# lasgroup/safe-adaptation-gym

Measured on AMD Instinct MI355X. Metric: env-steps/sec (batched) Point/GoToGoal, higher is better.
Workload: dtype f32

## Files before the change

### safe_adaptation_gym_amd/csrc/sag_api.hip

```cpp
#include <hip/hip_runtime.h>

#include <cmath>
#include <cstdarg>
#include <cstdio>
#include <cstdlib>
#include <algorithm>
#include <cstring>
#include <string>
#include <vector>

#include "sag_device.hpp"
#include "sag_reset.hpp"
#include "sag_rollout.hpp"
#include "sag_fork.hpp"

#ifndef SAG_SPLIT_MIN_ENVS
#define SAG_EARLY_FORK_MIN_ENVS 2097152
#define SAG_SPLIT_MIN_ENVS 262144
#define SAG_SPLIT_MIN_ENVS_CAR 393216
#endif

using namespace sag;

namespace {
// ... 340 lines not shown

void launch_lidar_cost(sag_ctx* c, int n, int K, const float* d_robot, const float* d_pts, const uint8_t* d_grp, float hazard_size,
                       float* d_lid, int32_t* d_bins, uint8_t* d_cost) {
  static const bool use_reg = [] { const char* e = getenv("SAG_LIDAR_REG"); return !e || atoi(e) != 0; }();
  int team = n <= 16384 ? 16 : (n <= 262144 ? 8 : 4);
  if (const char* e = getenv("SAG_LIDAR_TEAM")) team = atoi(e);
  if (team == 2)
    hipLaunchKernelGGL(k_lidar_cost_team<2>, dim3((n + 31) / 32), dim3(WAVE), 0, c->stream, n, K, d_robot, d_pts, d_grp, hazard_size,
                       d_lid, d_bins, d_cost);
  else if (team == 8)
    hipLaunchKernelGGL(k_lidar_cost_team<8>, dim3((n + 7) / 8), dim3(WAVE), 0, c->stream, n, K, d_robot, d_pts, d_grp, hazard_size,
                       d_lid, d_bins, d_cost);
  else if (team >= 16)
    hipLaunchKernelGGL(k_lidar_cost_team<16>, dim3((n + 3) / 4), dim3(WAVE), 0, c->stream, n, K, d_robot, d_pts, d_grp, hazard_size,
                       d_lid, d_bins, d_cost);
  else if (team >= 4)
    hipLaunchKernelGGL(k_lidar_cost_team<4>, dim3((n + 15) / 16), dim3(WAVE), 0, c->stream, n, K, d_robot, d_pts, d_grp, hazard_size,
                       d_lid, d_bins, d_cost);
  else if (K <= LC_KREG && use_reg)
    hipLaunchKernelGGL(k_lidar_cost_reg, dim3((n + WAVE - 1) / WAVE), dim3(WAVE), 0, c->stream, n, K, d_robot, d_pts, d_grp,
                       hazard_size, d_lid, d_bins, d_cost);
  else
    hipLaunchKernelGGL(k_lidar_cost, dim3((n + WAVE - 1) / WAVE), dim3(WAVE), lidar_cost_lds_bytes(K), c->stream, n, K, d_robot, d_pts,
                       d_grp, hazard_size, d_lid, d_bins, d_cost);
}

}

extern "C" {

int sag_device_count(void) {
  int n = 0;
  if (hipGetDeviceCount(&n) != hipSuccess) return 0;
  return n;
}

int sag_robot_info(int32_t robot, int32_t out[5], double* dt) {
  if (robot < 0 || robot > 2 || !out || !dt) return SAG_ERR_ARG;
  const RobotInfo& r = ROBOTS[robot];
  out[0] = r.nu; out[1] = r.obs_dim; out[2] = r.nstep; out[3] = r.nq; out[4] = r.nv;
  *dt = r.dt;
  return SAG_OK;
}

const char* sag_last_error(const sag_ctx* ctx) { return ctx ? ctx->err.c_str() : g_create_error.c_str(); }

int sag_create(const sag_config* cfg, sag_ctx** out) {
  if (!cfg || !out) return fail(nullptr, SAG_ERR_ARG, "null argument");
  *out = nullptr;
  if (cfg->abi_version != SAG_ABI_VERSION)
    return fail(nullptr, SAG_ERR_ARG, "ABI version %d, library is %d", cfg->abi_version, SAG_ABI_VERSION);
  if (cfg->robot < 0 || cfg->robot > 2) return fail(nullptr, SAG_ERR_ARG, "bad robot %d", cfg->robot);
  if (cfg->n_envs <= 0) return fail(nullptr, SAG_ERR_ARG, "n_envs must be positive");
  if (cfg->max_hazards < 0 || cfg->max_hazards > SAG_MAX_HAZARDS || cfg->max_vases < 0 ||
      cfg->max_vases > SAG_MAX_VASES || cfg->max_pillars < 0 || cfg->max_pillars > SAG_MAX_PILLARS ||
      cfg->max_buttons < 0 || cfg->max_buttons > SAG_MAX_BUTTONS)
    return fail(nullptr, SAG_ERR_ARG, "capacity out of range");
  int ndev = 0;
  if (hipGetDeviceCount(&ndev) != hipSuccess || ndev == 0)
    return fail(nullptr, SAG_ERR_NODEVICE, "no HIP device visible");
  if (cfg->device < 0 || cfg->device >= ndev)
    return fail(nullptr, SAG_ERR_NODEVICE, "device %d out of range (%d visible)", cfg->device, ndev);
  sag_ctx* c = new sag_ctx();
  c->cfg = *cfg; c->rb = ROBOTS[cfg->robot]; c->N = cfg->n_envs;
  c->split = c->N >= (cfg->robot == SAG_ROBOT_CAR ? SAG_SPLIT_MIN_ENVS_CAR : SAG_SPLIT_MIN_ENVS);
  if (const char* e = getenv("SAG_SPLIT")) c->split = atoi(e) != 0;
  const size_t N = (size_t)c->N;
#define CREATE_CHK(call)                                                                         \
  do {                                                                                           \
    hipError_t e_ = (call);                                                                      \
    if (e_ != hipSuccess) {                                                                      \
      int rc_ = fail(nullptr, SAG_ERR_HIP, "%s failed: %s", #call, hipGetErrorString(e_));       \
      sag_destroy(c);                                                                            \
      return rc_;                                                                                \
    }                                                                                            \
  } while (0)
  CREATE_CHK(hipSetDevice(cfg->device));
  CREATE_CHK(hipStreamCreateWithFlags(&c->stream, hipStreamNonBlocking));
  {
    int lo = 0, hi = 0;
    CREATE_CHK(hipDeviceGetStreamPriorityRange(&lo, &hi));
    CREATE_CHK(hipStreamCreateWithPriority(&c->stream2, hipStreamNonBlocking, lo));
  }
  CREATE_CHK(hipEventCreateWithFlags(&c->ev_fork, hipEventDisableTiming));
  CREATE_CHK(hipEventCreateWithFlags(&c->ev_join, hipEventDisableTiming));
  CREATE_CHK(hipEventCreateWithFlags(&c->ev_xsrc, hipEventDisableTiming));
  CREATE_CHK(hipEventCreateWithFlags(&c->ev_xdone, hipEventDisableTiming));
  if (const char* e = getenv("SAG_EARLY_FORK")) c->early_fork = atoi(e);
  if (const char* e = getenv("SAG_BUSY_KINDS")) c->busy_kinds = atoi(e) != 0 ? 1 : 0;
  if (const char* e = getenv("SAG_BUSY_KINDS_MIN")) c->kinds_min = atoi(e);
  {
    hipDeviceProp_t prop;
    if (hipGetDeviceProperties(&prop, cfg->device) == hipSuccess && prop.multiProcessorCount > 0) c->n_cu = prop.multiProcessorCount;
  }
  CREATE_CHK(hipMalloc(&c->S, N * DEV_FLOATS * sizeof(float)));
  CREATE_CHK(hipMalloc(&c->I, icount(N) * sizeof(int32_t)));
  CREATE_CHK(hipMalloc(&c->G, N * 3 * NBODY * sizeof(float)));
  CREATE_CHK(hipMalloc(&c->d_rows, BUSY_CLASSES * N * sizeof(int32_t)));
  CREATE_CHK(hipMalloc(&c->d_kind, N));
  CREATE_CHK(hipMemset(c->d_kind, 0, N));
  CREATE_CHK(hipMalloc(&c->d_count, (2 * BUSY_CLASSES + 1) * sizeof(int32_t)));
  CREATE_CHK(hipMemset(c->d_count, 0, (2 * BUSY_CLASSES + 1) * sizeof(int32_t)));
  CREATE_CHK(hipMalloc(&c->L_f, N * SAG_REC_FLOATS * sizeof(float)));
  CREATE_CHK(hipMalloc(&c->L_i, N * SAG_REC_INTS * sizeof(int32_t)));
  CREATE_CHK(hipMalloc(&c->st_f, N * SAG_REC_FLOATS * sizeof(float)));
  CREATE_CHK(hipMalloc(&c->st_i, N * SAG_REC_INTS * sizeof(int32_t)));
// ... 748 lines not shown
```

### safe_adaptation_gym_amd/csrc/sag_device.hpp

```cpp
#pragma once
#include <hip/hip_runtime.h>
#include <stdint.h>

#include <type_traits>

#include "../../include/sag.h"

namespace sag {

constexpr int WAVE = 64;

enum { DI_META = 0, DI_TSTATE = 1, DI_STEP = 2, DI_ENVID = 3, DI_FLAGS = 4, DI_COUNT = 5 };
constexpr int FLAG_EPISODE_SHIFT = 8;
__host__ __device__ constexpr size_t ipad(size_t N) { return (N + 3) & ~(size_t)3; }
__host__ __device__ constexpr size_t icount(size_t N) { return ipad(N) + 4 * N; }
__host__ __device__ constexpr size_t iaddr(int w, size_t N, size_t i) {
  return w == DI_TSTATE ? i : ipad(N) + i * 4 + (w == DI_META ? 0 : (w == DI_STEP ? 1 : (w == DI_ENVID ? 2 : 3)));
}

constexpr int DEV_FLOATS = 192, DEV_GROUPS = DEV_FLOATS / 4;
constexpr int DV_POS = 40, DV_VEL = 76, DG_HAZ = 5, DG_POS = 10, DG_PILLARS = 4, DG_BUTTONS = 28;
__host__ __device__ constexpr int didx(int k) {
  return k < 6 ? k
       : k < 9 ? 136 + (k - 6)
// ... 454 lines not shown
    const float ha = a.box ? a.b : a.a;
    const float lax = obx + a.ox * rc - a.oy * rs, lay = oby + a.ox * rs + a.oy * rc;
    const float pbx = a.a * ac + ha * as + SAT_EPS, pby = a.a * as + ha * ac + SAT_EPS;
#pragma unroll
    for (int gb = 0; gb < NB; gb++) {
      const Geom b = shape_geom(shB, gb, vsz, rstatic);
      const float hb = b.box ? b.b : b.a;
      const bool hit = !(fabsf(lbx[gb] - a.ox) > a.a + pax[gb]) && !(fabsf(lby[gb] - a.oy) > ha + pay[gb]) &&
                       !(fabsf(lax - b.ox) > b.a + pbx) && !(fabsf(lay - b.oy) > hb + pby);
      mask |= (mask_t)hit << (8 * ga + gb);
    }
  }
  int n = 0;
  while (mask) {
    const int pbit = (NA > 4 ? __ffsll((unsigned long long)mask) : __ffs((unsigned int)mask)) - 1;
    mask &= mask - 1;
    const int ga = NA > 1 ? pbit >> 3 : 0, gb = NB > 1 ? pbit & 7 : 0;
    const Geom a = shape_geom(SHA, ga, vsz, rstatic);
    Geom b = shape_geom(shB, gb, vsz, rstatic);
    const float ax = A.x + ca * a.ox - sa * a.oy, ay = A.y + sa * a.ox + ca * a.oy;
    const float qx = B.x + cb * b.ox - sb * b.oy, qy = B.y + sb * b.ox + cb * b.oy;
    if (!a.box && !b.box) n += cc_contact(A, B, ax, ay, a.a, qx, qy, b.a, sol);
    else if (!a.box) n += cb_contact(A, B, ax, ay, a.a, qx, qy, cb, sb, b.a, b.b, true, sol);
    else if (!b.box) n += cb_contact(B, A, qx, qy, b.a, ax, ay, ca, sa, a.a, a.b, false, sol);
    else n += bb_contact(A, B, ax, ay, ca, sa, a.a, a.b, qx, qy, cb, sb, b.a, b.b, sol);
  }
  return n;
}
template <int SHA, bool MULTI>
__device__ inline int collide_list(BV& A, float ca, float sa, BV& B, int shB, float cb, float sb, float vsz,
                                   float rstatic, const Sol& sol) {
#ifdef SAG_COLLIDE_REF
  return collide_shapes<true>(A, SHA, ca, sa, B, shB, cb, sb, vsz, rstatic, sol);
#endif
  if constexpr (MULTI) {
    if (shape_ngeom(shB) > 1) return collide_list_nb<SHA, 5>(A, ca, sa, B, SH_BOX, cb, sb, vsz, rstatic, sol);
  }
  if constexpr (SHA != SH_CAR) return collide_shapes<true>(A, SHA, ca, sa, B, shB, cb, sb, vsz, rstatic, sol);
  return collide_list_nb<SHA, 1>(A, ca, sa, B, shB, cb, sb, vsz, rstatic, sol);
}

constexpr int NBODY = SAG_MAX_VASES + 1, BOX_ID = SAG_MAX_VASES;
constexpr int DPOOL = 3;
enum { LS_X = 0, LS_Y = NBODY, LS_YAW = 2 * NBODY, LS_POOL = 3 * NBODY };
constexpr int LDS_SLOTS = LS_POOL + 6 * DPOOL;
constexpr int LDS_FLOATS = LDS_SLOTS * WAVE;
constexpr int CAR_PARK_SLOTS = 23;
enum { CP_FL = 0, CP_F0 = 5, CP_PX = 8, CP_EACC = 11, CP_Q = 16, CP_TAIL = 20 };
#define CPK(j) lds[(LDS_SLOTS + (j)) * WAVE + lane]
constexpr int STG_BASE = LS_YAW * WAVE;

enum { CY_LOAD = 0, CY_ROBOT, CY_RS, CY_RV, CY_VS, CY_VV_BROAD, CY_VV_NARROW, CY_INTEG, CY_WRITEBACK,
       CY_REWARD, CY_RESAMPLE, CY_COST, CY_LIDAR, CY_OBS_STORE, CY_TAIL, CY_N };
#ifdef SAG_WAVE_TIMES
constexpr int WT_MAX = 16384;
static __device__ unsigned long long g_wt[WT_MAX][2];
static __device__ int g_wt_env[WT_MAX][64];
static __device__ unsigned char g_wt_work[WT_MAX][64][8];
static __device__ unsigned short g_wt_trips[WT_MAX][8];
#define WTW(k) do { if (wt_work[k] < 255) wt_work[k]++; } while (0)
__device__ inline int wt_wave_max(int v) { for (int off = 32; off; off >>= 1) v = max(v, __shfl_xor(v, off)); return v; }
#define WTT(k, v) do { wt_trips[k] += (unsigned)wt_wave_max((int)(v)); } while (0)
#else
#define WTW(k) do {} while (0)
#define WTT(k, v) do {} while (0)
#endif
#ifdef SAG_CYCLES
static __device__ unsigned long long g_cyc[3][CY_N + 1];
static __device__ unsigned long long g_cyc_worst[3][CY_N + 1];
static __device__ unsigned long long g_cyc_worst_block[3];
static __device__ unsigned long long g_cyc_hist[3][64];
#define CYC_DECL unsigned long long cyc_acc[CY_N] = {}; unsigned long long cyc_t = __builtin_readcyclecounter();
#define CYC(k) do { const unsigned long long t_ = __builtin_readcyclecounter(); cyc_acc[k] += t_ - cyc_t; cyc_t = t_; } while (0)
__device__ inline unsigned long long cyc_wave_red(unsigned long long v, bool take_max) {
  for (int off = 32; off; off >>= 1) {
    const unsigned long long o = ((unsigned long long)(unsigned)__shfl_xor((int)(v >> 32), off) << 32) | (unsigned)__shfl_xor((int)(v & 0xffffffffu), off);
    v = take_max ? (o > v ? o : v) : (o < v ? o : v);
  }
  return v;
}
#define CYC_FLUSH(mode) do { unsigned long long tot_ = 0, red_[CY_N]; \
    for (int k_ = 0; k_ < CY_N; k_++) { red_[k_] = cyc_wave_red(k_ == CY_ROBOT && !live ? ~0ull : cyc_acc[k_], k_ != CY_ROBOT); tot_ += red_[k_]; } \
    if (lane == 0) { for (int k_ = 0; k_ < CY_N; k_++) atomicAdd(&g_cyc[mode][k_], red_[k_]); \
    atomicAdd(&g_cyc[mode][CY_N], 1ull); \
    { const int lg_ = 63 - __clzll((long long)(tot_ | 1ull)); const int q_ = lg_ >= 2 ? (int)(tot_ >> (lg_ - 2) & 3ull) : 0; \
      const int b_ = 4 * lg_ + q_ - 40; atomicAdd(&g_cyc_hist[mode][b_ < 0 ? 0 : (b_ > 63 ? 63 : b_)], 1ull); } \
    if (atomicMax(&g_cyc_worst[mode][CY_N], tot_) < tot_) { for (int k_ = 0; k_ < CY_N; k_++) g_cyc_worst[mode][k_] = red_[k_]; g_cyc_worst_block[mode] = blockIdx.x; } } } while (0)
#else
#define CYC_DECL
#define CYC(k) do {} while (0)
#define CYC_FLUSH(mode) do {} while (0)
#endif
}
#include "sag_doggo.hpp"
namespace sag {
#define SF(k) S[saddr((k), (size_t)N, (size_t)i)]
#define SD(d) S[((size_t)((d) >> 2) * N + i) * 4 + ((d) & 3)]
#define LP(base, k) lds[((base) + (k)) * WAVE + lane]
#define POOL(d, c) lds[(LS_POOL + (d) * 6 + (c)) * WAVE + lane]
#define STG(j) lds[STG_BASE + lane * STG_STRIDE + (j)]
#define TILE(b) lds[STG_BASE + (b) * WAVE + lane]

constexpr uint32_t TS_AWAKE_SHIFT = 17, TS_AWAKE_BITS = (1u << NBODY) - 1;

struct Dyn {
  float* lds; float* S; float* G; int lane, N, i;
  uint32_t dmap;
  uint32_t ovf;
  int nd;
  __device__ int vel_field(int k) const { return DV_VEL + 3 * k; }
  __device__ int slot(int k) const { return (int)(dmap >> (2 * k) & 3u) - 1; }
  __device__ bool has(int k) const { return (dmap >> (2 * k) & 3u) || (ovf >> k & 1u); }
  __device__ void ensure(int k, bool from_state) {
    if (has(k)) return;
    float vx = 0, vy = 0, w = 0;
    if (nd < DPOOL) {
      if (from_state) { const int f = vel_field(k); vx = SD(f); vy = SD(f + 1); w = SD(f + 2); }
      const int d = nd++;
      dmap |= (uint32_t)(d + 1) << (2 * k);
      POOL(d, 0) = vx; POOL(d, 1) = vy; POOL(d, 2) = w; POOL(d, 3) = 0; POOL(d, 4) = 0; POOL(d, 5) = 0;
    } else {
      ovf |= 1u << k;
      if (!from_state) { const int f = vel_field(k); SD(f) = 0; SD(f + 1) = 0; SD(f + 2) = 0; }
      for (int c = 0; c < 3; c++) G[((size_t)c * NBODY + k) * N + i] = 0;
    }
  }
  __device__ void get(int k, float& vx, float& vy, float& w, float& ax, float& ay, float& aw) const {
    const int d = slot(k);
    if (d >= 0) { vx = POOL(d, 0); vy = POOL(d, 1); w = POOL(d, 2); ax = POOL(d, 3); ay = POOL(d, 4); aw = POOL(d, 5); }
    else if (ovf >> k & 1u) {
      const int f = vel_field(k);
      vx = SD(f); vy = SD(f + 1); w = SD(f + 2);
      ax = G[((size_t)0 * NBODY + k) * N + i]; ay = G[((size_t)1 * NBODY + k) * N + i]; aw = G[((size_t)2 * NBODY + k) * N + i];
    } else { vx = vy = w = ax = ay = aw = 0; }
  }
  __device__ void set_acc(int k, float ax, float ay, float aw) {
    const int d = slot(k);
    if (d >= 0) { POOL(d, 3) = ax; POOL(d, 4) = ay; POOL(d, 5) = aw; }
    else { G[((size_t)0 * NBODY + k) * N + i] = ax; G[((size_t)1 * NBODY + k) * N + i] = ay; G[((size_t)2 * NBODY + k) * N + i] = aw; }
  }
  __device__ void set_vel(int k, float vx, float vy, float w) {
    const int d = slot(k);
    if (d >= 0) { POOL(d, 0) = vx; POOL(d, 1) = vy; POOL(d, 2) = w; }
    else { const int f = vel_field(k); SD(f) = vx; SD(f + 1) = vy; SD(f + 2) = w; }
  }
};

struct BodyK { int sh; float m, I, reff; };

struct LidarHit { int bin; float alias, sensor; };

__device__ __attribute__((noinline)) LidarHit lidar_exact(float rxf, float ryf, float yawf, float px, float py) {
// ... 88 lines not shown
  if (!is_task_obj || bk.sh == SH_BOX) {
    const float mm = !is_task_obj ? vk.m : bk.m, II = !is_task_obj ? vk.I : bk.I, rr = !is_task_obj ? vk.reff : bk.reff;
    const float fmax_ = MU * GRAV * mm;
    float fx = -SOL_D0 * mm * (bc * vx_ + ax_), fy = -SOL_D0 * mm * (bc * vy_ + ay_);
    const float f2 = fx * fx + fy * fy;
    if (f2 > fmax_ * fmax_) { const float sc = fmax_ / sqrtf(f2); fx *= sc; fy *= sc; }
    ax_ += fx / mm; ay_ += fy / mm;
    const float t = clampf(-SOL_D0 * II * (bc * w_ + aw_), -fmax_ * rr, fmax_ * rr);
    aw_ += t / II;
  } else {
    float c, s; sincosf(B[2], &s, &c);
    float bvx = c * vx_ + s * vy_, bvy = -s * vx_ + c * vy_, bax = c * ax_ + s * ay_, bay = -s * ax_ + c * ay_;
    const float mg = bk.m * GRAV;
    float tlim;
    if (bk.sh == SH_ROD) {
      const float mx = 1.5f * bk.m, lx = 0.05f * mg / 0.08f, ly = 1.2f * mg;
      const float fx = clampf(-SOL_D0 * mx * (bc * bvx + bax), -lx, lx);
      const float fy = clampf(-SOL_D0 * bk.m * (bc * bvy + bay), -ly, ly);
      bax += fx / mx; bay += fy / bk.m;
      tlim = 1.2f * mg * 0.15f;
    } else {
      const float me = 1.4f * bk.m, lim = 0.05f * mg / 0.14f;
      float fx = -SOL_D0 * me * (bc * bvx + bax), fy = -SOL_D0 * me * (bc * bvy + bay);
      const float f2 = fx * fx + fy * fy;
      if (f2 > lim * lim) { const float sc = lim / sqrtf(f2); fx *= sc; fy *= sc; }
      bax += fx / me; bay += fy / me;
      tlim = 0.003f * mg;
    }
    ax_ = c * bax - s * bay; ay_ = s * bax + c * bay;
    aw_ += clampf(-SOL_D0 * bk.I * (bc * w_ + aw_), -tlim, tlim) / bk.I;
  }
  vx_ += h * ax_; vy_ += h * ay_; w_ += h * aw_;
  if (fabsf(vx_) < REST_V && fabsf(vy_) < REST_V && fabsf(w_) < REST_W && fabsf(h * ax_) < REST_V &&
      fabsf(h * ay_) < REST_V && fabsf(h * aw_) < REST_W) { vx_ = 0; vy_ = 0; w_ = 0; }
  B[3] = vx_; B[4] = vy_; B[5] = w_;
  B[0] += h * vx_; B[1] += h * vy_; B[2] += h * w_;
}


enum { MODE_ALL = 0, MODE_QUIET = 1, MODE_BUSY = 2, MODE_POST = 3 };

constexpr int obs_dim(int robot) { return robot == SAG_ROBOT_DOGGO ? 104 : (robot == SAG_ROBOT_CAR ? 72 : 60); }
constexpr int quiet_lds_rows_chunked(int robot) { return LS_YAW + (robot == SAG_ROBOT_CAR ? 25 : 17); }
constexpr int quiet_lds_total(int robot) {
  const int own = quiet_lds_rows_chunked(robot) * WAVE * (int)sizeof(float), busy = (LDS_FLOATS + WAVE) * (int)sizeof(float);
  return busy > own ? own + (busy - own + 511) / 512 * 512 : own;
}
constexpr bool obs_whole_rows(int robot, bool has_btn, bool has_tbox, int mode) {
  const int cols = obs_dim(robot) - 16;
  return robot != SAG_ROBOT_DOGGO && mode != MODE_POST && !has_btn && !has_tbox && cols - 16 >= 2 * NBODY &&
         cols <= LDS_SLOTS &&
         cols * WAVE * (int)sizeof(float) <= quiet_lds_total(robot);
}
constexpr int quiet_lds_rows(int robot, bool has_btn, bool has_tbox) {
  const int chunked = quiet_lds_rows_chunked(robot), whole = obs_dim(robot) - 16;
  return obs_whole_rows(robot, has_btn, has_tbox, MODE_QUIET) && whole > chunked ? whole : chunked;
}
constexpr uint32_t TS_BUSY_BIT = 1u << 28;
constexpr int BUSY_CLASSES = 8;
__host__ __device__ constexpr int busy_class_order(int k) {
  constexpr int order[BUSY_CLASSES] = {7, 5, 3, 1, 6, 4, 2, 0};
  return order[k];
}

inline CarFricK car_fric_constants(float h) {
  CarFricK k;
  constexpr float CM = CAR_M, CIO = CAR_IO, COY = CAR_OY, CRW = 0.05f, AB = -CM * COY;
  constexpr float IDC = 1.0f / (CM * (CM * CIO - AB * AB));
  constexpr float M0 = (CM * CIO) * IDC, M2 = (-AB * CM) * IDC, M3 = (CM * CIO - AB * AB) * IDC, M5 = (CM * CM) * IDC;
  k.iIw = 1.0f / (CAR_IW + h * 0.001f); k.iIb = 1.0f / (CAR_IB + h * 0.001f);
  const float spw = CRW * CRW * k.iIw, spb = CRW * CRW * k.iIb;
  const float A_L = M3 + M5 * 0.13f * 0.13f + spw, A_T = M0 - 2 * M2 * 0.1f + M5 * 0.1f * 0.1f;
  const float A_X = M0 + 2 * M2 * 0.1f + M5 * 0.1f * 0.1f + spb, A_Y = M3 + spb;
  constexpr float RF = (1.0f - SOL_D0) / SOL_D0;
  k.R_L = A_L * RF; k.R_T = 0.5f * A_T * RF; k.R_X = A_X * RF; k.R_Y = A_Y * RF;
  k.iA_L = 1.0f / (A_L + k.R_L); k.iA_T = 1.0f / (A_T + k.R_T); k.iA_X = 1.0f / (A_X + k.R_X); k.iA_Y = 1.0f / (A_Y + k.R_Y);
  k.w_L = 1.0f / (spw + k.R_L); k.w_T = 1.0f / k.R_T; k.w_X = 1.0f / (spb + k.R_X); k.w_Y = 1.0f / (spb + k.R_Y);
  k.K00 = CM + k.w_T + k.w_X; k.K02 = AB - 0.1f * k.w_T + 0.1f * k.w_X;
  k.K22 = CIO + 0.13f * 0.13f * (k.w_L + k.w_L) + 0.1f * 0.1f * k.w_T + 0.1f * 0.1f * k.w_X;
  k.idk = 1.0f / (k.K00 * k.K22 - k.K02 * k.K02);
  k.iK11 = 1.0f / (CM + k.w_L + k.w_L + k.w_Y);
  return k;
}

template <int ROBOT, bool HAS_BTN, bool HAS_TBOX, int MODE>
__device__ __forceinline__ void step_body(const StepArgs& p, float* lds, const int lane, const int i,
                                          const bool live, const int base_env, const int nvalid,
                                          const uint64_t skip_mask, const int* rows) {
  constexpr int NSTAT = SAG_MAX_PILLARS + (HAS_BTN ? SAG_MAX_BUTTONS : 0);
  constexpr bool CAR = ROBOT == SAG_ROBOT_CAR, DOGGO = ROBOT == SAG_ROBOT_DOGGO;
  static_assert(!DOGGO || MODE == MODE_ALL || MODE == MODE_POST, "Doggo runs the single-launch form");
  static_assert(DOGGO || MODE != MODE_POST, "MODE_POST is the Doggo post kernel");
  constexpr bool QUIET = MODE == MODE_QUIET;
  constexpr bool PARK = CAR && !QUIET;
  constexpr int SH_ME = CAR ? SH_CAR : SH_ROBOT;
  constexpr int OBS_DIM = DOGGO ? 104 : (CAR ? 72 : 60);
  constexpr int NSENS = DOGGO ? 28 : OBS_DIM - 48, NCHUNK = DOGGO ? 5 : 4;
  constexpr int STG_STRIDE = DOGGO ? 29 : (CAR ? 25 : 17);
  static_assert(STG_BASE + WAVE * STG_STRIDE <= LDS_FLOATS, "staging tile must fit");
  CYC_DECL
  const float my_bound = shape_bound(SH_ME, 0.f, 0.f);
  const int N = p.N;
  float* __restrict__ S = p.S;
  int32_t* __restrict__ I = p.I;
  const int capV = p.max_vases, capH = p.max_hazards, capP = p.max_pillars, capB = HAS_BTN ? p.max_buttons : 0;

  const float4* __restrict__ S4 = reinterpret_cast<const float4*>(S);
  auto G4 = [&](int g) { return S4[(size_t)g * N + i]; };
  const bool use_hot = MODE == MODE_BUSY && p.hot != nullptr;
  const float4* __restrict__ H4 = use_hot ? reinterpret_cast<const float4*>(p.hot) + (size_t)i * HOT_GROUPS : nullptr;
  auto GH = [&](int g, int hslot) { return use_hot ? H4[hslot] : G4(g); };
  int4 iw;
  uint32_t tstate;
  if (use_hot) {
    const float4 hi = H4[14], ht = H4[15];
    iw = make_int4(__float_as_int(hi.x), __float_as_int(hi.y), __float_as_int(hi.z), __float_as_int(hi.w));
    tstate = (uint32_t)__float_as_int(ht.x);
  } else {
    iw = reinterpret_cast<const int4*>(I + ipad((size_t)N))[i];
    tstate = (uint32_t)I[iaddr(DI_TSTATE, (size_t)N, (size_t)i)];
  }
  const uint32_t meta = (uint32_t)iw.x;
  int step = iw.y;
  const uint32_t env_id = (uint32_t)iw.z;
  const float4 gA = GH(0, 0), gB = GH(1, 1), gC = GH(2, 2), gD = GH(3, 3);
  BV R;
  R.x = gA.x; R.y = gA.y;
  float yaw = gA.z;
  R.vx = gA.w; R.vy = gB.x; R.w = gB.y;
  R.ax = R.ay = R.aw = 0; R.dyn = 1;
  const float gear = gC.y, damp = gC.z;
  const float vsz = gD.z, psz = gD.w;
  float ext[9] = {0, 0, 0, 0, 0, 1, 0, 0, 0}, eacc[5] = {0, 0, 0, 0, 0};
  constexpr int DG_EXT = (152 >> 2);
  static_assert(didx(SAG_F_ROBOT_EXT) == 152 && didx(SAG_F_ROBOT_EXT + 8) == 160, "car extension = device groups 38..40");
  float4 ext_tail = make_float4(0.f, 0.f, 0.f, 0.f);
  if constexpr (CAR) {
    const float4 e0 = G4(DG_EXT), e1 = G4(DG_EXT + 1);
    ext_tail = G4(DG_EXT + 2);
    ext[0] = e0.x; ext[1] = e0.y; ext[2] = e0.z; ext[3] = e0.w; ext[4] = e1.x; ext[5] = e1.y; ext[6] = e1.z; ext[7] = e1.w;
    ext[8] = ext_tail.x;
    if constexpr (PARK) {
      CPK(CP_Q) = ext[5]; CPK(CP_Q + 1) = ext[6]; CPK(CP_Q + 2) = ext[7]; CPK(CP_Q + 3) = ext[8];
      CPK(CP_TAIL) = ext_tail.y; CPK(CP_TAIL + 1) = ext_tail.z; CPK(CP_TAIL + 2) = ext_tail.w;
    }
  }
  float goalx = gB.z, goaly = gB.w;
  float last0 = gC.x;
  float a0 = 0, a1 = 0, n0 = 0, n1 = 0;
  if (!p.observe_only) {
    if constexpr (!DOGGO) {
      const float2 a = reinterpret_cast<const float2*>(p.actions)[i];
      a0 = a.x; a1 = a.y;
      if (p.noise) { const float2 z = reinterpret_cast<const float2*>(p.noise)[i]; n0 = z.x; n1 = z.y; }
    }
  }
  {
    float vpos[36];
    const int need = HAS_TBOX && p.has_box ? 9 : (3 * capV + 3) / 4;
#pragma unroll
    for (int g = 0; g < 9; g++) {
      float4 v = make_float4(0.f, 0.f, 0.f, 0.f);
      if (g < need) v = GH(DG_POS + g, 5 + g);
      vpos[4 * g] = v.x; vpos[4 * g + 1] = v.y; vpos[4 * g + 2] = v.z; vpos[4 * g + 3] = v.w;
    }
#pragma unroll
    for (int k = 0; k < SAG_MAX_VASES; k++)
      if (k >= capV) { vpos[3 * k] = vpos[3 * k + 1] = vpos[3 * k + 2] = 0; }
    if (!(HAS_TBOX && p.has_box)) { vpos[3 * BOX_ID] = vpos[3 * BOX_ID + 1] = vpos[3 * BOX_ID + 2] = 0; }
#pragma unroll
    for (int k = 0; k < NBODY; k++) { LP(LS_X, k) = vpos[3 * k]; LP(LS_Y, k) = vpos[3 * k + 1]; LP(LS_YAW, k) = vpos[3 * k + 2]; }
  }
  float stx[NSTAT], sty[NSTAT];
  {
    float4 v = make_float4(0.f, 0.f, 0.f, 0.f);
    if (capP > 0) v = GH(DG_PILLARS, 4);
    stx[0] = v.x; sty[0] = v.y; stx[1] = capP > 1 ? v.z : 0.f; sty[1] = capP > 1 ? v.w : 0.f;
    static_assert(SAG_MAX_PILLARS == 2, "pillars fill one group");
  }
  if constexpr (HAS_BTN) {
    float bt[12];
#pragma unroll
    for (int g = 0; g < 3; g++) {
      float4 v = make_float4(0.f, 0.f, 0.f, 0.f);
      if (2 * g < capB) v = G4(DG_BUTTONS + g);
      bt[4 * g] = v.x; bt[4 * g + 1] = v.y; bt[4 * g + 2] = v.z; bt[4 * g + 3] = v.w;
    }
    static_assert(SAG_MAX_BUTTONS == 6, "buttons fill three groups");
#pragma unroll
    for (int k = 0; k < SAG_MAX_BUTTONS; k++) {
      stx[SAG_MAX_PILLARS + k] = k < capB ? bt[2 * k] : 0.f;
      sty[SAG_MAX_PILLARS + k] = k < capB ? bt[2 * k + 1] : 0.f;
    }
  }
  const int task = meta & 15, nH = meta >> 4 & 15, nV = meta >> 8 & 15, nP = meta >> 12 & 3,
            nB = HAS_BTN ? (meta >> 14 & 7) : 0, box_kind = HAS_TBOX ? (meta >> 17 & 3) : 0;
  const bool has_box = HAS_TBOX && box_kind != SAG_BOX_NONE;
  auto is_box = [](int k) { return HAS_TBOX && k == BOX_ID; };
  int flags = 0;

  Rng rng;
  rng.tape = p.tape ? p.tape + (size_t)i * p.tape_len : nullptr;
  rng.len = p.tape_len; rng.pos = 0; rng.exhausted = 0;
  rng.k0 = p.key0; rng.k1 = p.key1; rng.env = env_id; rng.step = (uint32_t)step;
  rng.ep4 = ((uint32_t)iw.w >> FLAG_EPISODE_SHIFT) << 2;

  float ctrl0 = 0, ctrl1 = 0;
  float ctrl12[DOGGO ? 12 : 1] = {};
  if constexpr (DOGGO) {
    if (!p.observe_only) {
      const float an = SF(SAG_F_ACTION_NOISE);
#pragma unroll 1
      for (int j = 0; j < 12; j += 2) {
        float z0, z1;
        if (p.noise) { z0 = p.noise[(size_t)i * 12 + j]; z1 = p.noise[(size_t)i * 12 + j + 1]; }
        else {
          uint32_t c[4] = {rng.env, rng.step, (uint32_t)(j >> 1), rng.ep4 | 1u};
          philox4x32_10(c, p.key0, p.key1);
          box_muller(c[0], c[1], z0, z1);
        }
        const float l0 = SF(SAG_F_CTRL_SCALE + j), l1 = SF(SAG_F_CTRL_SCALE + j + 1);
        ctrl12[j] = clampf(p.actions[(size_t)i * 12 + j] + an * z0, -l0, l0);
        ctrl12[j + 1] = clampf(p.actions[(size_t)i * 12 + j + 1] + an * z1, -l1, l1);
      }
    }
  }
  if (!p.observe_only) {
    if (!p.noise && !DOGGO) {
      uint32_t c[4] = {rng.env, rng.step, 0u, rng.ep4 | 1u};
      philox4x32_10(c, p.key0, p.key1);
      box_muller(c[0], c[1], n0, n1);
    }
    const float an = gC.w;
    const float cs0 = gD.x, cs1 = gD.y;
    ctrl0 = clampf(a0 + an * n0, -cs0, cs0);
    ctrl1 = clampf(a1 + an * n1, -cs1, cs1);
    if (task == SAG_TASK_CATCH_GOAL) {
      int t = tstate >> 7 & 15;
      t = t - 1 > 0 ? t - 1 : 0;
      float cur = SF(SAG_F_CATCH + 2), nxt = SF(SAG_F_CATCH + 3);
      if (t == 0) {
        cur = nxt;
        nxt = (float)rng.uniform(0.2, 1.0);
        if (rng.exhausted) flags |= 2;
        if (live) { SF(SAG_F_CATCH + 2) = cur; SF(SAG_F_CATCH + 3) = nxt; }
// ... 519 lines not shown
    const float dth = (fmaxf(fabsf(R.w), 3.0f) + 1.0f) * T;
    const float fa = 0.1f + reach, fb = 0.0707107f + reach + 0.1f * dth;
    const float Bx = R.x + 0.1f * cy, By = R.y + 0.1f * sy;
#pragma unroll 1
    for (int k = 0; k < nV; k++) {
      const float vx_ = LP(LS_X, k), vy_ = LP(LS_Y, k);
      const float dx = vx_ - R.x, dyy = vy_ - R.y, rs = rr + vase_r;
      if (dx * dx + dyy * dyy <= rs * rs) {
        if constexpr (FINE) {
          float sv, cv; sincosf(LP(LS_YAW, k), &sv, &cv);
          auto box_d2 = [&](float px, float py) {
            const float wx = px - vx_, wy = py - vy_;
            const float ex = fmaxf(fabsf(cv * wx + sv * wy) - vsz, 0.f), ey = fmaxf(fabsf(cv * wy - sv * wx) - vsz, 0.f);
            return ex * ex + ey * ey;
          };
          busy |= box_d2(R.x, R.y) <= fa * fa || box_d2(Bx, By) <= fb * fb;
        } else busy = true;
      }
    }
    if (has_box) {
      const float dx = LP(LS_X, BOX_ID) - R.x, dyy = LP(LS_Y, BOX_ID) - R.y, rs = rr + box_r;
      near_obj = dx * dx + dyy * dyy <= rs * rs;
    }
#pragma unroll 1
    for (int k = 0; k < n_static; k++) {
      if (k == capP) k = SAG_MAX_PILLARS;
      const bool is_p = k < SAG_MAX_PILLARS;
      const bool on = is_p ? (k < nP) : (k - SAG_MAX_PILLARS < nB);
      const float sr = is_p ? psz : BUTTON_R;
      const float skx = pick(stx, k), sky = pick(sty, k);
      const float dx = skx - R.x, dyy = sky - R.y, rs = rr + sr;
      if constexpr (FINE) {
        const float ex = skx - Bx, ey = sky - By;
        near_static |= on && (dx * dx + dyy * dyy <= (fa + sr) * (fa + sr) || ex * ex + ey * ey <= (fb + sr) * (fb + sr));
      } else near_static |= on && dx * dx + dyy * dyy <= rs * rs;
    }
    const bool near_vase = busy && !moving;
    busy |= near_obj || near_static;
    const uint32_t kind = p.busy_kinds ? (uint32_t)near_obj | (uint32_t)near_static << 1 | (uint32_t)(near_vase || moving) << 2 : 0u;
    const uint32_t nbit = TS_BUSY_BIT << (p.phase ^ 1);
    tstate = busy ? (tstate | nbit) : (tstate & ~nbit);
    if (busy && live && p.kind) p.kind[i] = (uint8_t)kind;
    busy_next = busy;
  }

  CYC(CY_WRITEBACK);
  float hzx[SAG_MAX_HAZARDS], hzy[SAG_MAX_HAZARDS];
  float hsz;
  {
    float hz[20];
#pragma unroll
    for (int g = 0; g < 5; g++) {
      float4 v = make_float4(0.f, 0.f, 0.f, 0.f);
      if (g == 4 || 2 * g < capH) v = use_hot ? reinterpret_cast<const float4*>(p.hot_haz)[(size_t)i * 5 + g] : G4(DG_HAZ + g);
      hz[4 * g] = v.x; hz[4 * g + 1] = v.y; hz[4 * g + 2] = v.z; hz[4 * g + 3] = v.w;
    }
    static_assert(SAG_MAX_HAZARDS == 9, "hazards + size fill five groups");
#pragma unroll
    for (int k = 0; k < SAG_MAX_HAZARDS; k++) { hzx[k] = k < capH ? hz[2 * k] : 0.f; hzy[k] = k < capH ? hz[2 * k + 1] : 0.f; }
    hsz = hz[18];
  }

  bool bad = false;
  {
    float v[6] = {R.x, R.y, yaw, R.vx, R.vy, R.w};
#pragma unroll
    for (int k = 0; k < 6; k++) bad |= !(fabsf(v[k]) <= 1e10f);
    if constexpr (DOGGO) {
      bad |= !(fabs(dgs.pos[2]) <= 1e10) || !(fabs(dgs.vlin[2]) <= 1e10);
      for (int k = 0; k < 4; k++) bad |= !(fabs(dgs.quat[k]) <= 1e10);
      for (int k = 0; k < 3; k++) bad |= !(fabs(dgs.wloc[k]) <= 1e10);
      for (int k = 0; k < DG_NJ; k++) bad |= !(fabs(dgs.q[k]) <= 1e10) || !(fabs(dgs.qd[k]) <= 1e10);
    }
  }

  double rew0 = 0, rew1 = 0;
  int met = 0;
  const double rx = R.x, ry = R.y;
  bool need_goal = false;
  float box_last1 = 0, box_last2 = 0;
  if (!p.observe_only && !bad) {
    if (task == SAG_TASK_PRESS_BUTTONS || task == SAG_TASK_PRESS_BUTTONS_SCARCE) {
      int gb = tstate & 7, bstate = tstate >> 3 & 1, timer = tstate >> 4 & 7;
      double gd = dist2d(rx, ry, SD(112 + 2 * gb), SD(113 + 2 * gb));
      double r = task == SAG_TASK_PRESS_BUTTONS ? (double)last0 - gd : 0.0;
      float last = (float)gd;
      if (btn_mask >> gb & 1) {
        r += 1.0; met = 1;
        gb = (int)(rng.word() & 3u);
        if (rng.exhausted) flags |= 2;
        timer = 5;
        last = (float)dist2d(rx, ry, SD(112 + 2 * gb), SD(113 + 2 * gb));
        bstate = 0;
      }
      if (bstate == 0) {
        if (timer != 0) timer -= 1;
        else { bstate = 1; timer = 5; }
      }
      last0 = last;
      tstate = (tstate & ~127u) | (uint32_t)gb | (uint32_t)bstate << 3 | (uint32_t)timer << 4;
      rew0 = r;
    } else if (task == SAG_TASK_COLLECT) {
      uint32_t act = tstate >> 11 & 63;
      if (act == 0) act = (1u << nB) - 1;
      uint32_t hit = act & btn_mask;
      if (hit) {
        rew0 = 1.0; met = 1;
        act &= ~(hit & (0u - hit));
      }
      tstate = (tstate & ~(63u << 11)) | act << 11;
    } else if (!has_box) {
      double gx = goalx, gy = goaly;
      double dx = rx - gx, dyy = ry - gy, dz = (DOGGO ? (double)(float)dgs.pos[2] : (double)PT_Z) - GOAL_Z;
      double dist = sqrt(dx * dx + dyy * dyy + dz * dz);
// ... 380 lines not shown
  if (live) {
    if (p.reward) {
      float2 r;
      r.x = bad ? -10.0f : (float)rew0; r.y = bad ? 0.0f : (float)rew1;
      reinterpret_cast<float2*>(p.reward)[i] = r;
    }
    if (p.cost) p.cost[i] = (uint8_t)cost;
    if (p.done) p.done[i] = bad ? 1 : 0;
    if (p.goal_met) p.goal_met[i] = (uint8_t)met;
    if (p.tape_used) p.tape_used[i] = rng.pos;
  }
  CYC(CY_TAIL);
  CYC_FLUSH(MODE);
#ifdef SAG_WAVE_TIMES
  if (MODE == MODE_BUSY && blockIdx.x < WT_MAX) {
    g_wt_env[blockIdx.x][lane] = live ? i : -1;
    for (int k = 0; k < 8; k++) g_wt_work[blockIdx.x][lane][k] = (unsigned char)wt_work[k];
    if (lane == 0) for (int k = 0; k < 8; k++) g_wt_trips[blockIdx.x][k] = (unsigned short)wt_trips[k];
  }
#endif
}

template <int ROBOT, bool HAS_BTN, bool HAS_TBOX>
__global__ __launch_bounds__(WAVE, SAG_STEP_MIN_WAVES) void k_step(StepArgs p) {
  __shared__ float lds[LDS_FLOATS + (ROBOT == SAG_ROBOT_CAR ? CAR_PARK_SLOTS * WAVE : 0)];
  static_assert(ROBOT != SAG_ROBOT_DOGGO, "Doggo: k_doggo_physics + k_step_doggo_post");
  const int epw = p.envs_per_wave;
  const int lane = threadIdx.x, base = blockIdx.x * epw, gi = base + lane;
  const bool live = gi < p.N && lane < epw;
  step_body<ROBOT, HAS_BTN, HAS_TBOX, MODE_ALL>(p, lds, lane, live ? gi : p.N - 1, live, base,
                                                 min(epw, p.N - base), 0ull, nullptr);
}

template <bool HAS_BTN, bool HAS_TBOX>
__global__ __launch_bounds__(WAVE, 1) void k_step_doggo_post(StepArgs p) {
  __shared__ float lds[LDS_FLOATS];
  const int lane = threadIdx.x, base = blockIdx.x * WAVE, gi = base + lane;
  const bool live = gi < p.N;
  step_body<SAG_ROBOT_DOGGO, HAS_BTN, HAS_TBOX, MODE_POST>(p, lds, lane, live ? gi : p.N - 1, live, base, min(WAVE, p.N - base),
                                                            0ull, nullptr);
}

#ifndef SAG_QUIET_MIN_WAVES
#define SAG_QUIET_MIN_WAVES 4
#endif
#ifndef SAG_CAR_QUIET_MIN_WAVES
#define SAG_CAR_QUIET_MIN_WAVES 3
#endif
template <int ROBOT, bool HAS_BTN, bool HAS_TBOX>
__global__ __launch_bounds__(WAVE, ROBOT == SAG_ROBOT_CAR ? SAG_CAR_QUIET_MIN_WAVES : SAG_QUIET_MIN_WAVES) void k_step_quiet(StepArgs p) {
  constexpr int QSLOTS = quiet_lds_rows(ROBOT, HAS_BTN, HAS_TBOX);
  static_assert(QSLOTS >= LS_YAW + NBODY, "the yaw rows written at load time must stay in bounds");
  static_assert(QSLOTS * WAVE * (int)sizeof(float) <= quiet_lds_total(ROBOT), "the quiet array stays inside the footprint of its launch");
  __shared__ float lds[QSLOTS * WAVE];
  const int lane = threadIdx.x, base = blockIdx.x * WAVE, gi = base + lane;
  const bool in = gi < p.N;
  const bool busy = in && ((uint32_t)p.I[iaddr(DI_TSTATE, (size_t)p.N, (size_t)gi)] & (TS_BUSY_BIT << p.phase));
  const uint64_t skip = __ballot(busy || !in);
  if (skip == ~0ull) return;
  const bool live = in && !busy;
  step_body<ROBOT, HAS_BTN, HAS_TBOX, MODE_QUIET>(p, lds, lane, in ? gi : p.N - 1, live, base,
                                                   min(WAVE, p.N - base), skip, nullptr);
}

constexpr int COMPACT_PER_LANE = 16, COMPACT_ENVS = 256 * COMPACT_PER_LANE;
template <bool KINDS>
__global__ __launch_bounds__(256) void k_compact(const int32_t* I, const uint8_t* kind, int N, int phase, int32_t* rows, int32_t* count,
                                                  int32_t* zero_for_next, const int32_t* prev_total, int kinds_min) {
  constexpr int NC = KINDS ? BUSY_CLASSES : 1;
  const bool use_kinds = KINDS && *prev_total > kinds_min;
  if (blockIdx.x == 0 && threadIdx.x < BUSY_CLASSES) zero_for_next[threadIdx.x] = 0;
  __shared__ int wave_tot[4][BUSY_CLASSES];
  __shared__ int wave_base[4][BUSY_CLASSES];
  const int lane = threadIdx.x & 63, wv = threadIdx.x >> 6;
  const int e0 = blockIdx.x * COMPACT_ENVS + wv * (WAVE * COMPACT_PER_LANE);
  uint32_t bmask = 0;
  uint64_t kinds = 0;
  int pre[COMPACT_PER_LANE];
  int run[BUSY_CLASSES] = {};
  uint32_t tw[COMPACT_PER_LANE];
  uint8_t kb[COMPACT_PER_LANE];
#pragma unroll
  for (int j = 0; j < COMPACT_PER_LANE; j++) {
    const int e = e0 + j * WAVE + lane;
    tw[j] = e < N ? (uint32_t)I[iaddr(DI_TSTATE, (size_t)N, (size_t)e)] : 0u;
    kb[j] = KINDS && e < N && use_kinds ? kind[e] : (uint8_t)0;
  }
#pragma unroll
  for (int j = 0; j < COMPACT_PER_LANE; j++) {
    const bool b = (tw[j] & (TS_BUSY_BIT << phase)) != 0;
    const int k = b ? (int)kb[j] & (BUSY_CLASSES - 1) : 0;
    bmask |= (uint32_t)b << j;
    kinds |= (uint64_t)k << (4 * j);
    pre[j] = 0;
#pragma unroll
    for (int c = 0; c < NC; c++) {
      const uint64_t m = __ballot(b && k == c);
      if (b && k == c) pre[j] = run[c] + __popcll(m & ((1ull << lane) - 1));
      run[c] += __popcll(m);
    }
  }
  if (lane == 0)
#pragma unroll
    for (int c = 0; c < NC; c++) wave_tot[wv][c] = run[c];
  __syncthreads();
  if (threadIdx.x < NC) {
    const int c = threadIdx.x;
    const int total = wave_tot[0][c] + wave_tot[1][c] + wave_tot[2][c] + wave_tot[3][c];
    int base = total ? atomicAdd(count + c, total) : 0;
// ... 490 lines not shown
```

Measured before the change: 4.834 billion.

## Issue quiet Point kernel loads before busy check and park hazards in LDS

```diff
diff --git a/safe_adaptation_gym_amd/csrc/sag_api.hip b/safe_adaptation_gym_amd/csrc/sag_api.hip
--- a/safe_adaptation_gym_amd/csrc/sag_api.hip
+++ b/safe_adaptation_gym_amd/csrc/sag_api.hip
@@ -416,6 +416,7 @@
     return fail(nullptr, SAG_ERR_ARG, "ABI version %d, library is %d", cfg->abi_version, SAG_ABI_VERSION);
   if (cfg->robot < 0 || cfg->robot > 2) return fail(nullptr, SAG_ERR_ARG, "bad robot %d", cfg->robot);
   if (cfg->n_envs <= 0) return fail(nullptr, SAG_ERR_ARG, "n_envs must be positive");
+  if (cfg->n_envs > (1 << 28)) return fail(nullptr, SAG_ERR_ARG, "n_envs above 2^28 is not supported");
   if (cfg->max_hazards < 0 || cfg->max_hazards > SAG_MAX_HAZARDS || cfg->max_vases < 0 ||
       cfg->max_vases > SAG_MAX_VASES || cfg->max_pillars < 0 || cfg->max_pillars > SAG_MAX_PILLARS ||
       cfg->max_buttons < 0 || cfg->max_buttons > SAG_MAX_BUTTONS)
diff --git a/safe_adaptation_gym_amd/csrc/sag_device.hpp b/safe_adaptation_gym_amd/csrc/sag_device.hpp
--- a/safe_adaptation_gym_amd/csrc/sag_device.hpp
+++ b/safe_adaptation_gym_amd/csrc/sag_device.hpp
@@ -530,6 +530,7 @@
 
 enum { CY_LOAD = 0, CY_ROBOT, CY_RS, CY_RV, CY_VS, CY_VV_BROAD, CY_VV_NARROW, CY_INTEG, CY_WRITEBACK,
        CY_REWARD, CY_RESAMPLE, CY_COST, CY_LIDAR, CY_OBS_STORE, CY_TAIL, CY_N };
+enum { CY_Q_HEAD = CY_RS, CY_Q_HAZ = CY_RV };
 #ifdef SAG_WAVE_TIMES
 constexpr int WT_MAX = 16384;
 static __device__ unsigned long long g_wt[WT_MAX][2];
@@ -550,6 +551,7 @@
 static __device__ unsigned long long g_cyc_hist[3][64];
 #define CYC_DECL unsigned long long cyc_acc[CY_N] = {}; unsigned long long cyc_t = __builtin_readcyclecounter();
 #define CYC(k) do { const unsigned long long t_ = __builtin_readcyclecounter(); cyc_acc[k] += t_ - cyc_t; cyc_t = t_; } while (0)
+#define CYC_ARRIVED(v) asm volatile("" :: "v"(v))
 __device__ inline unsigned long long cyc_wave_red(unsigned long long v, bool take_max) {
   for (int off = 32; off; off >>= 1) {
     const unsigned long long o = ((unsigned long long)(unsigned)__shfl_xor((int)(v >> 32), off) << 32) | (unsigned)__shfl_xor((int)(v & 0xffffffffu), off);
@@ -567,6 +569,7 @@
 #else
 #define CYC_DECL
 #define CYC(k) do {} while (0)
+#define CYC_ARRIVED(v) do {} while (0)
 #define CYC_FLUSH(mode) do {} while (0)
 #endif
 }
@@ -576,6 +579,7 @@
 #define SD(d) S[((size_t)((d) >> 2) * N + i) * 4 + ((d) & 3)]
 #define LP(base, k) lds[((base) + (k)) * WAVE + lane]
 #define POOL(d, c) lds[(LS_POOL + (d) * 6 + (c)) * WAVE + lane]
+#define HZP(j) (*((j) < HAZ_PARK_STATIC ? &lds[(LS_POOL + (j)) * WAVE + lane] : &hz_dyn[((j) - HAZ_PARK_STATIC) * WAVE + lane]))
 #define STG(j) lds[STG_BASE + lane * STG_STRIDE + (j)]
 #define TILE(b) lds[STG_BASE + (b) * WAVE + lane]
 
@@ -770,6 +774,12 @@
          cols <= LDS_SLOTS &&
          cols * WAVE * (int)sizeof(float) <= quiet_lds_total(robot);
 }
+constexpr int HAZ_PARK_ROWS = 2 * SAG_MAX_HAZARDS + 1;
+constexpr int HAZ_PARK_STATIC = obs_dim(SAG_ROBOT_POINT) - 16 - LS_POOL;
+constexpr bool quiet_one_phase(int robot, bool has_btn, bool has_tbox) {
+  return robot == SAG_ROBOT_POINT && obs_whole_rows(robot, has_btn, has_tbox, MODE_QUIET) && HAZ_PARK_STATIC > 0 &&
+         (obs_dim(robot) - 16 + HAZ_PARK_ROWS - HAZ_PARK_STATIC) * WAVE * (int)sizeof(float) <= quiet_lds_total(robot);
+}
 constexpr int quiet_lds_rows(int robot, bool has_btn, bool has_tbox) {
   const int chunked = quiet_lds_rows_chunked(robot), whole = obs_dim(robot) - 16;
   return obs_whole_rows(robot, has_btn, has_tbox, MODE_QUIET) && whole > chunked ? whole : chunked;
@@ -803,13 +813,14 @@
 
 template <int ROBOT, bool HAS_BTN, bool HAS_TBOX, int MODE>
 __device__ __forceinline__ void step_body(const StepArgs& p, float* lds, const int lane, const int i,
-                                          const bool live, const int base_env, const int nvalid,
-                                          const uint64_t skip_mask, const int* rows) {
+                                          const bool live_arg, const int base_env, const int nvalid,
+                                          const uint64_t skip_arg, const int* rows) {
   constexpr int NSTAT = SAG_MAX_PILLARS + (HAS_BTN ? SAG_MAX_BUTTONS : 0);
   constexpr bool CAR = ROBOT == SAG_ROBOT_CAR, DOGGO = ROBOT == SAG_ROBOT_DOGGO;
   static_assert(!DOGGO || MODE == MODE_ALL || MODE == MODE_POST, "Doggo runs the single-launch form");
   static_assert(DOGGO || MODE != MODE_POST, "MODE_POST is the Doggo post kernel");
   constexpr bool QUIET = MODE == MODE_QUIET;
+  constexpr bool ONE_PHASE = QUIET && quiet_one_phase(ROBOT, HAS_BTN, HAS_TBOX);
   constexpr bool PARK = CAR && !QUIET;
   constexpr int SH_ME = CAR ? SH_CAR : SH_ROBOT;
   constexpr int OBS_DIM = DOGGO ? 104 : (CAR ? 72 : 60);
@@ -824,7 +835,15 @@
   const int capV = p.max_vases, capH = p.max_hazards, capP = p.max_pillars, capB = HAS_BTN ? p.max_buttons : 0;
 
   const float4* __restrict__ S4 = reinterpret_cast<const float4*>(S);
-  auto G4 = [&](int g) { return S4[(size_t)g * N + i]; };
+  const uint32_t voff = (uint32_t)i << 4;
+  auto G4 = [&](int g) {
+    if constexpr (ONE_PHASE) return *reinterpret_cast<const float4*>(reinterpret_cast<const char*>(S4 + (size_t)g * N) + voff);
+    else return S4[(size_t)g * N + i];
+  };
+  auto G4sel = [&](bool on, int g) {
+    const float4 v = G4(on ? g : 0);
+    return on ? v : make_float4(0.f, 0.f, 0.f, 0.f);
+  };
   const bool use_hot = MODE == MODE_BUSY && p.hot != nullptr;
   const float4* __restrict__ H4 = use_hot ? reinterpret_cast<const float4*>(p.hot) + (size_t)i * HOT_GROUPS : nullptr;
   auto GH = [&](int g, int hslot) { return use_hot ? H4[hslot] : G4(g); };
@@ -834,6 +853,10 @@
     const float4 hi = H4[14], ht = H4[15];
     iw = make_int4(__float_as_int(hi.x), __float_as_int(hi.y), __float_as_int(hi.z), __float_as_int(hi.w));
     tstate = (uint32_t)__float_as_int(ht.x);
+  } else if constexpr (ONE_PHASE) {
+    tstate = *reinterpret_cast<const uint32_t*>(reinterpret_cast<const char*>(I) + (voff >> 2));
+    iw = *reinterpret_cast<const int4*>(reinterpret_cast<const char*>(I + ipad((size_t)N)) + voff);
+    static_assert(iaddr(DI_TSTATE, 8, 5) == 5, "TSTATE is the plain [N] column in front");
   } else {
     iw = reinterpret_cast<const int4*>(I + ipad((size_t)N))[i];
     tstate = (uint32_t)I[iaddr(DI_TSTATE, (size_t)N, (size_t)i)];
@@ -868,31 +891,38 @@
   float a0 = 0, a1 = 0, n0 = 0, n1 = 0;
   if (!p.observe_only) {
     if constexpr (!DOGGO) {
-      const float2 a = reinterpret_cast<const float2*>(p.actions)[i];
+      float2 a;
+      if constexpr (ONE_PHASE) a = *reinterpret_cast<const float2*>(reinterpret_cast<const char*>(p.actions) + (voff >> 1));
+      else a = reinterpret_cast<const float2*>(p.actions)[i];
       a0 = a.x; a1 = a.y;
       if (p.noise) { const float2 z = reinterpret_cast<const float2*>(p.noise)[i]; n0 = z.x; n1 = z.y; }
     }
   }
+  float vpos[36];
   {
-    float vpos[36];
     const int need = HAS_TBOX && p.has_box ? 9 : (3 * capV + 3) / 4;
 #pragma unroll
     for (int g = 0; g < 9; g++) {
       float4 v = make_float4(0.f, 0.f, 0.f, 0.f);
-      if (g < need) v = GH(DG_POS + g, 5 + g);
+      if constexpr (ONE_PHASE) v = G4sel(g < need, DG_POS + g);
+      else if (g < need) v = GH(DG_POS + g, 5 + g);
       vpos[4 * g] = v.x; vpos[4 * g + 1] = v.y; vpos[4 * g + 2] = v.z; vpos[4 * g + 3] = v.w;
     }
 #pragma unroll
     for (int k = 0; k < SAG_MAX_VASES; k++)
       if (k >= capV) { vpos[3 * k] = vpos[3 * k + 1] = vpos[3 * k + 2] = 0; }
     if (!(HAS_TBOX && p.has_box)) { vpos[3 * BOX_ID] = vpos[3 * BOX_ID + 1] = vpos[3 * BOX_ID + 2] = 0; }
+  }
+  auto positions_to_lds = [&]() {
 #pragma unroll
     for (int k = 0; k < NBODY; k++) { LP(LS_X, k) = vpos[3 * k]; LP(LS_Y, k) = vpos[3 * k + 1]; LP(LS_YAW, k) = vpos[3 * k + 2]; }
-  }
+  };
+  if constexpr (!ONE_PHASE) positions_to_lds();
   float stx[NSTAT], sty[NSTAT];
   {
     float4 v = make_float4(0.f, 0.f, 0.f, 0.f);
-    if (capP > 0) v = GH(DG_PILLARS, 4);
+    if constexpr (ONE_PHASE) v = G4sel(capP > 0, DG_PILLARS);
+    else if (capP > 0) v = GH(DG_PILLARS, 4);
     stx[0] = v.x; sty[0] = v.y; stx[1] = capP > 1 ? v.z : 0.f; sty[1] = capP > 1 ? v.w : 0.f;
     static_assert(SAG_MAX_PILLARS == 2, "pillars fill one group");
   }
@@ -909,6 +939,28 @@
     for (int k = 0; k < SAG_MAX_BUTTONS; k++) {
       stx[SAG_MAX_PILLARS + k] = k < capB ? bt[2 * k] : 0.f;
       sty[SAG_MAX_PILLARS + k] = k < capB ? bt[2 * k + 1] : 0.f;
+    }
+  }
+  bool live = live_arg;
+  uint64_t skip_mask = skip_arg;
+  if constexpr (ONE_PHASE) {
+    HIP_DYNAMIC_SHARED(float, hz_dyn)
+    float4 hq[5];
+#pragma unroll
+    for (int g = 0; g < 5; g++) {
+      hq[g] = G4sel(g == 4 || 2 * g < capH, DG_HAZ + g);
+    }
+    asm volatile("" ::: "memory");
+    const bool busy = live_arg && (tstate & (TS_BUSY_BIT << p.phase));
+    skip_mask = __ballot(busy || !live_arg);
+    if (skip_mask == ~0ull) return;
+    live = live_arg && !busy;
+    CYC(CY_Q_HEAD);
+    positions_to_lds();
+#pragma unroll
+    for (int g = 0; g < 5; g++) {
+      HZP(4 * g) = hq[g].x; HZP(4 * g + 1) = hq[g].y; HZP(4 * g + 2) = hq[g].z;
+      if (4 * g + 3 < HAZ_PARK_ROWS) HZP(4 * g + 3) = hq[g].w;
     }
   }
   const int task = meta & 15, nH = meta >> 4 & 15, nV = meta >> 8 & 15, nP = meta >> 12 & 3,
@@ -1534,7 +1586,11 @@
 #pragma unroll
     for (int g = 0; g < 5; g++) {
       float4 v = make_float4(0.f, 0.f, 0.f, 0.f);
-      if (g == 4 || 2 * g < capH) v = use_hot ? reinterpret_cast<const float4*>(p.hot_haz)[(size_t)i * 5 + g] : G4(DG_HAZ + g);
+      if constexpr (ONE_PHASE) {
+        HIP_DYNAMIC_SHARED(float, hz_dyn)
+        v.x = HZP(4 * g); v.y = HZP(4 * g + 1); v.z = HZP(4 * g + 2);
+        if (4 * g + 3 < HAZ_PARK_ROWS) v.w = HZP(4 * g + 3);
+      } else if (g == 4 || 2 * g < capH) v = use_hot ? reinterpret_cast<const float4*>(p.hot_haz)[(size_t)i * 5 + g] : G4(DG_HAZ + g);
       hz[4 * g] = v.x; hz[4 * g + 1] = v.y; hz[4 * g + 2] = v.z; hz[4 * g + 3] = v.w;
     }
     static_assert(SAG_MAX_HAZARDS == 9, "hazards + size fill five groups");
@@ -1542,6 +1598,7 @@
     for (int k = 0; k < SAG_MAX_HAZARDS; k++) { hzx[k] = k < capH ? hz[2 * k] : 0.f; hzy[k] = k < capH ? hz[2 * k + 1] : 0.f; }
     hsz = hz[18];
   }
+  if constexpr (QUIET) { CYC_ARRIVED(hsz); CYC(CY_Q_HAZ); }
 
   bool bad = false;
   {
@@ -2028,9 +2085,14 @@
   constexpr int QSLOTS = quiet_lds_rows(ROBOT, HAS_BTN, HAS_TBOX);
   static_assert(QSLOTS >= LS_YAW + NBODY, "the yaw rows written at load time must stay in bounds");
   static_assert(QSLOTS * WAVE * (int)sizeof(float) <= quiet_lds_total(ROBOT), "the quiet array stays inside the footprint of its launch");
+  static_assert(!quiet_one_phase(ROBOT, HAS_BTN, HAS_TBOX) || QSLOTS == LS_POOL + HAZ_PARK_STATIC, "parked hazards end with the static array");
   __shared__ float lds[QSLOTS * WAVE];
   const int lane = threadIdx.x, base = blockIdx.x * WAVE, gi = base + lane;
   const bool in = gi < p.N;
+  if constexpr (quiet_one_phase(ROBOT, HAS_BTN, HAS_TBOX)) {
+    step_body<ROBOT, HAS_BTN, HAS_TBOX, MODE_QUIET>(p, lds, lane, in ? gi : p.N - 1, in, base, min(WAVE, p.N - base), 0ull, nullptr);
+    return;
+  }
   const bool busy = in && ((uint32_t)p.I[iaddr(DI_TSTATE, (size_t)p.N, (size_t)gi)] & (TS_BUSY_BIT << p.phase));
   const uint64_t skip = __ballot(busy || !in);
   if (skip == ~0ull) return;
```

Measured after the change: 4.550 billion. -5.9%, worse.
